# ska-telescope/ska-sdp-screen-fitting

Measured on AMD Instinct MI355X. Metric: screen-slots/sec (ant×time×freq) + FITS-cube wall-clock, KL 256² screen, higher is better.
Workload: dtype f64

## Files before the change

include/screenfit.h:

```cpp
#ifndef SCREENFIT_H
#define SCREENFIT_H

#include <stddef.h>
#include <stdint.h>

#ifdef __cplusplus
extern "C" {
#endif

#define SF_OK 0
#define SF_EINVAL (-22)
#define SF_ENOMEM (-12)
#define SF_EIO (-5)
#define SF_ENODEV (-19)

#define SF_MAX_DIR 60
#define SF_MAX_FIT_DIR 128
#define SF_MAX_EVAL_DIR 128

#define SF_SCREEN_PHASE 0
#define SF_SCREEN_TEC 1
#define SF_SCREEN_AMPLITUDE 2

#define SF_EVAL_NAN_SCRUB 1u
// ... 32 lines not shown
#define SF_OPT_EVAL_XCD_MAP 7
#define SF_OPT_EVAL_GROUPS 8
#define SF_OPT_EVAL_BANDS 9
#define SF_OPT_FIT_LEAN 10
#define SF_OPT_TESS_SLOTS 11
#define SF_OPT_TESS_WAVES 12
#define SF_OPT_TESS_TILE 13
#define SF_OPT_TESS_BOX 14
#define SF_OPT_EVAL_INT 15
#define SF_OPT_EVAL_WG_WAVES 16
#define SF_OPT_FIT_EIG_WAVES 17
#define SF_OPT_FIT_SUBSET_DELETION 18
#define SF_OPT_FIT_WIDE_CACHE 19
#define SF_OPT_FIT_WIDE_POOL_MB 20
#define SF_OPT_FIT_WIDE_POOL_MAX 21
#define SF_EVAL_KERNEL_AUTO 0
#define SF_EVAL_KERNEL_TILE 1
#define SF_EVAL_KERNEL_LDS4 2
#define SF_EVAL_KERNEL_LDS8 3
#define SF_EVAL_KERNEL_LDS16 4
#define SF_EVAL_KERNEL_LDS8H 5
#define SF_EVAL_KERNEL_LDS16H 6
#define SF_EVAL_KERNEL_TILE3 7
#define SF_EVAL_KERNEL_SHB 8
#define SF_EVAL_KERNEL_WIDE 9
int sf_get_eval_kernel(sf_ctx* ctx, int gain, unsigned flags, int* kernel);
#define SF_EVAL_CONTRACTION_F64 0
#define SF_EVAL_CONTRACTION_I8_DIGITS 1
int sf_get_eval_contraction(sf_ctx* ctx, int gain, unsigned flags, int* contraction);
int sf_set_option(sf_ctx* ctx, int option, int value);
// ... 6 lines not shown
                 double beta);
int sf_set_basis_wide(sf_ctx* ctx, const double* pp_host, int D, double r0,
                      double beta);
int sf_get_basis(sf_ctx* ctx, double* c_host, double* pinv_c_host,
                 double* u_host, double* eig_host);

int sf_set_piercepoints(sf_ctx* ctx, const double* pp_host, int D, double r0,
                        double beta);

int sf_kl_fit(sf_ctx* ctx, const double* phase, const float* weight, int T,
              int F, int A, const int* station_order_host,
              const sf_fit_params* params, double* coef, double* resid,
              float* w_out, int32_t* order_out);

int sf_get_fit_stats(sf_ctx* ctx, int* n_masks, int* n_general);

int sf_get_fit_pool(sf_ctx* ctx, uint64_t* masks_host, double* entries_host,
                    int max_masks, int* n_masks);
int sf_get_fit_pool_wide(sf_ctx* ctx, uint64_t* masks_host, double* entries_host,
                         int max_masks, int* n_masks);

int sf_set_grid(sf_ctx* ctx, const double* x_host, int nx,
                const double* y_host, int ny);

int sf_kl_eval(sf_ctx* ctx, const double* coef, int64_t S, float* out,
               int64_t ring_slots, unsigned flags);

int sf_kl_eval_gain(sf_ctx* ctx, const double* coef_phase,
                    const double* coef_xx, const double* coef_yy, int64_t S,
                    float* out, int64_t ring_slots, unsigned flags);
// ... 42 lines not shown
```

ska-sdp-screen-fitting_amd/csrc/capi.hip:

```cpp
#include <hip/hip_runtime.h>

#include <algorithm>
#include <cmath>
#include <cstring>
#include <string>
#include <vector>

#include "sf_internal.h"

namespace sf {
static thread_local std::string g_last_error;
void set_error(const std::string& msg) { g_last_error = msg; }
}

using sf::set_error;

namespace {

int check_device(int device) {
  int n = 0;
  hipError_t e = hipGetDeviceCount(&n);
  if (e != hipSuccess || n == 0) {
    set_error("no HIP device available");
    return SF_ENODEV;
// ... 105 lines not shown
  hipFree(ctx->d_pfrag);
  hipFree(ctx->d_cdig);
  hipFree(ctx->d_kdig);
  hipFree(ctx->d_kflag);
  if (ctx->kdig_read) (void)hipEventDestroy(ctx->kdig_read);
  hipFree(ctx->d_skip);
  hipFree(ctx->d_st_order);
  hipFree(ctx->d_keys);
  hipFree(ctx->d_ids);
  hipFree(ctx->d_pool_mask);
  hipFree(ctx->d_pool);
  hipFree(ctx->d_pool_status);
  hipFree(ctx->d_pos);
  hipFree(ctx->d_sigma);
  hipFree(ctx->d_class);
  hipFree(ctx->d_counters);
  hipFree(ctx->d_scratch);
  hipFree(ctx->d_wscratch);
  hipFree(ctx->d_oscratch);
  hipFree(ctx->d_gw);
  hipFree(ctx->d_smooth);
  hipFree(ctx->d_tess_tab);
  hipFree(ctx->d_tec_ch);
  hipFree(ctx->d_trash);
  delete ctx;
  return SF_OK;
}

int sf_set_stream(sf_ctx* ctx, void* stream) {
  SF_REQUIRE(ctx, SF_EINVAL, "sf_set_stream: NULL context");
// ... 44 lines not shown
  SF_REQUIRE(ctx, SF_EINVAL, "sf_set_option: NULL context");
  switch (option) {
    case SF_OPT_FIT_GENERAL:
      ctx->force_general = value != 0;
      return SF_OK;
    case SF_OPT_EVAL_KERNEL:
      SF_REQUIRE(value >= SF_EVAL_KERNEL_AUTO && value <= SF_EVAL_KERNEL_WIDE,
                 SF_EINVAL, "sf_set_option: unknown evaluation kernel");
      ctx->eval_kernel = value;
      return SF_OK;
    case SF_OPT_FIT_PACK:
      ctx->fit_pack = value != 0;
      return SF_OK;
    case SF_OPT_FIT_LEAN:
      ctx->fit_lean = value != 0;
      return SF_OK;
    case SF_OPT_EVAL_KS_PAD:
      SF_REQUIRE(value >= 0 && value <= 3, SF_EINVAL,
                 "sf_set_option: k-step padding must be 0..3");
      ctx->eval_ks_pad = value;
      return SF_OK;
    case SF_OPT_EVAL_SLEEP:
      SF_REQUIRE(value >= 0 && value <= 1000, SF_EINVAL,
                 "sf_set_option: eval sleep must be 0..1000");
      ctx->eval_sleep = value;
      return SF_OK;
    case SF_OPT_EVAL_XCD_MAP:
      SF_REQUIRE(value >= -1 && value <= 1, SF_EINVAL,
                 "sf_set_option: XCD map must be -1, 0 or 1");
      ctx->eval_xcd_map = value;
// ... 273 lines not shown
}

int sf_get_fit_stats(sf_ctx* ctx, int* n_masks, int* n_general) {
  SF_REQUIRE(ctx, SF_EINVAL, "sf_get_fit_stats: NULL context");
  int c[sf::kFitCounters] = {};
  SF_HIP(hipSetDevice(ctx->device));
  SF_HIP(hipStreamSynchronize(ctx->stream));
  if (ctx->d_counters)
    SF_HIP(hipMemcpy(c, ctx->d_counters, sizeof(c), hipMemcpyDeviceToHost));
  static_assert(sf::kCntIds == sf::kCntWideDecomp, "n_masks reads one slot");
  if (n_masks) *n_masks = c[sf::kCntIds];
  if (n_general) *n_general = c[sf::kCntSlow];
  return SF_OK;
}

int sf_get_fit_pool(sf_ctx* ctx, uint64_t* masks_host, double* entries_host,
                    int max_masks, int* n_masks) {
  SF_REQUIRE(ctx && n_masks && max_masks >= 0, SF_EINVAL, "sf_get_fit_pool: bad argument");
  SF_REQUIRE(max_masks == 0 || (masks_host && entries_host), SF_EINVAL,
             "sf_get_fit_pool: NULL output");
  SF_REQUIRE(!ctx->wide, SF_EINVAL,
             "sf_get_fit_pool: 64-bit mask keys; above SF_MAX_DIR directions "
             "(sf_set_basis_wide) call sf_get_fit_pool_wide");
  SF_HIP(hipSetDevice(ctx->device));
  SF_HIP(hipStreamSynchronize(ctx->stream));
  int c0 = 0;
  if (ctx->d_counters)
    SF_HIP(hipMemcpy(&c0, ctx->d_counters + sf::kCntIds, sizeof(int),
                     hipMemcpyDeviceToHost));
  const int n = ctx->pool_D == ctx->D && (size_t)c0 <= ctx->pool_cap ? c0 : 0;
// ... 424 lines not shown
```

ska-sdp-screen-fitting_amd/csrc/kl_fit_fast.hip:

```cpp
#include <hip/hip_runtime.h>

#include <cmath>
#include <cstdlib>

#include "kl_fit_pool.h"
#include "kl_fit_steps.h"
#include "sf_internal.h"

namespace sf {

constexpr size_t kLdsBytes = 160 * 1024;
constexpr double kTinyW = kPinvAtol * 1.001;

template <int GW>
__global__ __launch_bounds__(256) void kl_classify_kernel(
    const float* __restrict__ weight, int64_t S, int F, int A, int D,
    const int* __restrict__ st_order, const uint8_t* __restrict__ skip,
    int ref_skip, unsigned long long* __restrict__ keys, int cap,
    int* __restrict__ pos, uint8_t* __restrict__ cls,
    int* __restrict__ counters,
    double* __restrict__ coef, double* __restrict__ resid,
    float* __restrict__ w_out, int32_t* __restrict__ order_out) {
  constexpr int kPerWave = 64 / GW;
  const int l = lane();
  const int g = l / GW;
  const int d = l % GW;
  const int64_t s = ((int64_t)blockIdx.x * (blockDim.x / 64) + threadIdx.x / 64) *
                        kPerWave + g;
  const bool live = s < S && d < D;
  float x = 0.0f;
  if (live) {
    x = weight[s * D + d];
    w_out[s * D + d] = x;
  }
  const unsigned long long bm = __ballot(live && x > 0.0f);
  const unsigned long long bt = __ballot(live && x > 0.0f && (double)x <= kTinyW);
  const unsigned long long gmask = (GW == 64) ? ~0ull : ((1ull << GW) - 1ull);
  const unsigned long long mask = (bm >> (g * GW)) & gmask;
  const bool tiny = ((bt >> (g * GW)) & gmask) != 0ull;
  const float w_first = __shfl(x, g * GW + (mask ? __builtin_ctzll(mask) : 0));
  const unsigned long long bn = __ballot(live && x > 0.0f && x != w_first);
  const bool nonuniform = ((bn >> (g * GW)) & gmask) != 0ull;
  if (s >= S) return;
  const SlotGeom sg(s, F, A);
  const bool skipped = sg.skipped(skip, ref_skip);
  if (live && skipped) {
    coef[s * D + d] = 0.0;
    resid[s * D + d] = 0.0;
  }
  if (d != 0) return;
  if (skipped) {
    cls[s] = 1;
    order_out[s] = 0;
    pos[s] = -2;
    return;
  }
  order_out[s] = st_order[sg.a];
  if (tiny) atomicAdd(counters + kCntSlow, 1);
  else if (nonuniform) atomicAdd(counters + kCntNonUniform, 1);
  cls[s] = tiny ? 2 : 0;
  if (mask == full_mask(D)) pos[s] = -1;
  else if (mask == 0ull) pos[s] = -2;
  else pos[s] = table_insert(keys, cap, mask);
}

struct FastLds {
  const double* U;
  const double* C;
  int cld;
  const double* lam;
  double* Vs;
  double* lams;
  double* G;
  double* M;
  double* vec;
// ... 176 lines not shown

#ifndef SF_FIT_MINW
#define SF_FIT_MINW 4
#endif
template <bool SLOW, int SPW, bool LEAN>
__global__ __launch_bounds__(256, SLOW ? 1 : SF_FIT_MINW) void kl_fit_pass_kernel(
    int it, int niter, int64_t S, int F, int A, int D,
    const double* __restrict__ phase, const double* __restrict__ refph,
    int ref_sub, const double* __restrict__ g_u, const double* __restrict__ g_c,
    const double* __restrict__ g_eig, const int* __restrict__ st_order,
    const uint8_t* __restrict__ cls, int* __restrict__ pos,
    const int* __restrict__ ids, unsigned long long* __restrict__ keys, int cap,
    const double* __restrict__ pool, int pool_cap, int* __restrict__ counters,
    int screen_type, double nsigma, int adjust_order, double* __restrict__ coef,
    double* __restrict__ resid, float* __restrict__ w_out,
    int32_t* __restrict__ order_out) {
#pragma clang fp contract(off)
  extern __shared__ double smem[];
  const int ld = odd_ld(D);
  using G = Group<SPW>;
  using M = FitMath<!SLOW>;
  const G tm;
  constexpr bool CG = SPW == 1;
  const int nwaves = blockDim.x / 64;
  const int nslots = nwaves * SPW;
  const int wv = (threadIdx.x / 64) * SPW + G::index();
  const int d = G::lane();
  double* sU = smem;
  double* sC = CG ? nullptr : sU + D * ld;
  double* sl = sU + (CG ? 1 : 2) * D * ld;
  for (int e = threadIdx.x; e < D * D; e += blockDim.x) {
// ... 13 lines not shown
    L.Vs = L.G = L.M = L.lams = nullptr;
    L.vec = wb;
    L.cs = nullptr;
    L.pr = nullptr;
  } else {
    L.Vs = wb;
    L.G = wb + D * ld;
    L.M = L.G + D * ld;
    L.lams = (SLOW ? L.M + D * ld : L.G + D * ld);
    L.vec = L.lams + 64;
    L.cs = reinterpret_cast<double2*>(L.vec + 6 * 64);
    L.pr = reinterpret_cast<int2*>(L.cs + 64);
  }
  const uint8_t want = SLOW ? 2 : 0;

  for (int64_t s = (int64_t)blockIdx.x * nslots + wv; s < S;
       s += (int64_t)gridDim.x * nslots) {
    if (SLOW && cls[s] != want) continue;
    const uint8_t cl = SLOW ? want : cls[s];
    const int a = (int)(s % A);
    const int p0 = pos[s];
    const int64_t base = s * D;
    double phi_d = 0.0, w_d = 0.0, white_d = 0.0, resid_d = 0.0;
    if (d < D) {
      phi_d = phase_ref(phase, refph, ref_sub, s, a, A, D, d);
      w_d = (double)w_out[base + d];
      white_d = it == 0 ? 0.0 : coef[base + d];
      resid_d = it == 0 ? 0.0 : resid[base + d];
    }
    double order = (double)order_out[s];
    const double station_order = (double)st_order[a];
    if (cl != want) continue;
// ... 150 lines not shown
    if (fabs(sd) > nsigma * sig && w != 0.0f) {
      w = 0.0f;
      w_out[s * D + d] = w;
      changed = true;
    }
    if (w > 0.0f) m |= 1ull << d;
  }
  if (changed) {
    pos[s] = (m == 0ull) ? -2 : (m == full_mask(D) ? -1 : table_insert(keys, cap, m));
  }
}

static int launch_pass(sf_ctx* ctx, bool slow, int it, const sf_fit_params* p,
                       const RefSpec& r, int64_t S, int F, int A,
                       const double* phase, double* coef, double* resid,
                       float* w_out, int32_t* order_out, bool lean) {
  const int D = ctx->D;
  const int spw = !slow && D <= 32 && ctx->fit_pack ? 2 : 1;
  lean = !slow && lean && ctx->fit_lean;
  decltype(&kl_fit_pass_kernel<false, 1, false>) const kernels[3][2] = {
      {kl_fit_pass_kernel<false, 1, false>, kl_fit_pass_kernel<false, 2, false>},
      {kl_fit_pass_kernel<false, 1, true>, kl_fit_pass_kernel<false, 2, true>},
      {kl_fit_pass_kernel<true, 1, false>, kl_fit_pass_kernel<true, 2, false>}};
  const auto kernel = kernels[slow ? 2 : lean][spw - 1];
  const size_t shared = fast_shared_bytes(D, spw == 1);
  const size_t slot = fast_wave_bytes(D, slow, lean);
  int nw = 1, best = 0;
  for (int k = 1; k <= 4; ++k) {
    const size_t per_wg = shared + (size_t)k * spw * slot;
    if (per_wg > kLdsBytes) break;
    const int waves = k * (int)(kLdsBytes / per_wg);
    if (waves > best) {
      best = waves;
      nw = k;
    }
  }
  const size_t shm = shared + (size_t)nw * spw * slot;
  SF_TRY_RC(allow_lds(kernel, shm));
  int64_t blocks = (S + nw * spw - 1) / (nw * spw);
  if (blocks > 16384) blocks = 16384;
  hipLaunchKernelGGL(kernel, dim3((unsigned)blocks), dim3(64 * nw), shm,
                     ctx->stream, it, p->niter, S, F, A, D, phase, r.refph, r.sub,
                     ctx->d_u, ctx->d_c, ctx->d_eig, ctx->d_st_order, ctx->d_class,
                     ctx->d_pos, ctx->d_ids, ctx->d_keys, (int)ctx->table_cap,
                     ctx->d_pool, (int)ctx->pool_cap, ctx->d_counters,
                     p->screen_type, p->nsigma, p->adjust_order, coef, resid, w_out,
                     order_out);
  SF_HIP(hipGetLastError());
  return SF_OK;
}

int launch_block_sigma(sf_ctx* ctx, int T, int F, int A, const double* phase,
                       const RefSpec& r, int screen_type, const double* resid,
                       const float* w_out) {
  hipLaunchKernelGGL(kl_block_sigma_kernel, dim3(F * A), dim3(256), 0,
                     ctx->stream, T, F, A, ctx->D, phase, r.refph, r.sub,
                     ctx->d_skip, r.skip, screen_type, resid, w_out,
                     ctx->d_sigma);
  SF_HIP(hipGetLastError());
  return SF_OK;
}

// ... 39 lines not shown
                              w_out, order_out);
  }
  SF_TRY_RC(fit_buffers(ctx, S, F, A, &resid, &w_out, &order_out));
  if (ctx->slot_cap < (size_t)S)
    SF_TRY_RC(replace_pair(ctx->slot_cap, (size_t)S, &ctx->d_pos, (size_t)S,
                           &ctx->d_class, (size_t)S));
  const size_t tcap = next_pow2((size_t)(2 * p->niter + 2) * (size_t)S + 64, 1);
  if (ctx->table_cap < tcap)
    SF_TRY_RC(replace_pair(ctx->table_cap, tcap, &ctx->d_keys, tcap, &ctx->d_ids, tcap));
  SF_TRY_RC(ensure_pool(ctx, 1024));
  const int cap = (int)ctx->table_cap;
  SF_HIP(hipMemsetAsync(ctx->d_keys, 0, ctx->table_cap * sizeof(unsigned long long),
                        ctx->stream));
  SF_HIP(hipMemsetAsync(ctx->d_ids, 0xff, ctx->table_cap * sizeof(int), ctx->stream));
  SF_HIP(hipMemsetAsync(ctx->d_counters, 0, kFitCounters * sizeof(int), ctx->stream));

  {
    const int gw = D <= 8 ? 8 : D <= 16 ? 16 : D <= 32 ? 32 : 64;
    const int64_t per_block = 4 * (64 / gw);
    const dim3 grid((unsigned)((S + per_block - 1) / per_block));
    const auto classify = gw == 8    ? kl_classify_kernel<8>
                          : gw == 16 ? kl_classify_kernel<16>
                          : gw == 32 ? kl_classify_kernel<32>
                                     : kl_classify_kernel<64>;
    hipLaunchKernelGGL(classify, grid, dim3(256), 0, ctx->stream, weight, S, F, A, D,
                       ctx->d_st_order, ctx->d_skip, r.skip, ctx->d_keys, cap,
                       ctx->d_pos, ctx->d_class, ctx->d_counters, coef, resid, w_out,
                       order_out);
    SF_HIP(hipGetLastError());
  }

  const bool block_flags = p->screen_type != SF_SCREEN_PHASE;
  for (int it = 0; it < p->niter; ++it) {
    int n_slow = 0, n_nonuniform = 0;
    SF_TRY_RC(number_and_decompose(ctx, &n_slow, &n_nonuniform));
    SF_TRY_RC(launch_pass(ctx, false, it, p, r, S, F, A, phase, coef, resid, w_out,
                          order_out, n_nonuniform == 0));
    if (n_slow > 0)
      SF_TRY_RC(launch_pass(ctx, true, it, p, r, S, F, A, phase, coef, resid, w_out,
                            order_out, false));
    if (block_flags && it + 1 < p->niter) {
      SF_TRY_RC(launch_block_sigma(ctx, T, F, A, phase, r, p->screen_type, resid,
                                 w_out));
      hipLaunchKernelGGL(kl_block_flag_kernel, dim3((unsigned)((S + 255) / 256)),
                         dim3(256), 0, ctx->stream, S, F, A, D, phase, r.refph,
                         r.sub, ctx->d_class, p->screen_type, p->nsigma,
                         ctx->d_sigma, resid, w_out, ctx->d_keys, cap,
                         ctx->d_pos);
      SF_HIP(hipGetLastError());
    }
  }
  int err = 0;
  SF_HIP(hipMemcpyAsync(&err, ctx->d_counters + kCntError, sizeof(int),
                        hipMemcpyDeviceToHost, ctx->stream));
  SF_HIP(hipStreamSynchronize(ctx->stream));
// ... 13 lines not shown
```

ska-sdp-screen-fitting_amd/csrc/kl_fit_masks.h:

```cpp
#pragma once

#include <hip/hip_runtime.h>

#include "sf_wave.h"

namespace sf {

__device__ __forceinline__ unsigned long long mix64(unsigned long long x) {
  x ^= x >> 30;
  x *= 0xbf58476d1ce4e5b9ull;
  x ^= x >> 27;
  x *= 0x94d049bb133111ebull;
  x ^= x >> 31;
  return x;
}

__host__ __device__ inline unsigned long long full_mask(int D) {
  return D == 64 ? ~0ull : (1ull << D) - 1ull;
}

inline size_t next_pow2(size_t x, size_t floor) {
  size_t p = floor;
  while (p < x) p <<= 1;
  return p;
}

__device__ __forceinline__ bool wave_in_table(int i, int cap) {
  return i - lane() < cap;
}

__device__ __forceinline__ int number_fresh(bool fresh, int* counter) {
  const unsigned long long nb = __ballot(fresh);
  if (nb == 0ull) return -1;
  int base = 0;
  if (lane() == 0) base = atomicAdd(counter, __popcll(nb));
  base = __shfl(base, 0);
  return fresh ? base + Group<1>::rank(nb) : -1;
}

}
```

ska-sdp-screen-fitting_amd/csrc/kl_fit_pool.h:

```cpp
#pragma once

#include <hip/hip_runtime.h>

#include <algorithm>

#include "kl_fit_masks.h"
#include "kl_fit_steps.h"
#include "sf_internal.h"

namespace sf {

constexpr unsigned long long kEmptyKey = 0ull;

__device__ int table_insert(unsigned long long* keys, int cap,
                            unsigned long long key) {
  int h = (int)(mix64(key) & (unsigned long long)(cap - 1));
  for (int probe = 0; probe < cap; ++probe) {
    unsigned long long prev = keys[h];
    if (prev == kEmptyKey) prev = atomicCAS(keys + h, kEmptyKey, key);
    if (prev == kEmptyKey || prev == key) return h;
    h = (h + 1) & (cap - 1);
  }
  return -3;
}

__device__ int table_find(const unsigned long long* keys, int cap,
                          unsigned long long key) {
  int h = (int)(mix64(key) & (unsigned long long)(cap - 1));
  for (int probe = 0; probe < cap; ++probe) {
    const unsigned long long k = keys[h];
    if (k == key) return h;
    if (k == kEmptyKey) return -1;
    h = (h + 1) & (cap - 1);
  }
  return -1;
}

__global__ __launch_bounds__(256) void kl_assign_kernel(
    const unsigned long long* __restrict__ keys, int cap, int* __restrict__ ids,
// ... 444 lines not shown
```

ska-sdp-screen-fitting_amd/csrc/sf_internal.h:

```cpp
#pragma once

#include <hip/hip_runtime.h>

#include <cstdint>
#include <string>
#include <vector>

#include "screenfit.h"

namespace sf {

void set_error(const std::string& msg);

#define SF_HIP(call)                                                        \
  do {                                                                      \
    hipError_t e_ = (call);                                                 \
    if (e_ != hipSuccess) {                                                 \
      ::sf::set_error(std::string(#call) + ": " + hipGetErrorString(e_));   \
      return SF_EIO;                                                        \
    }                                                                       \
  } while (0)

#define SF_REQUIRE(cond, code, msg) \
  do {                              \
// ... 48 lines not shown
  if (shm > 64 * 1024)
    SF_HIP(hipFuncSetAttribute(reinterpret_cast<const void*>(kernel),
                               hipFuncAttributeMaxDynamicSharedMemorySize, (int)shm));
  return SF_OK;
}

enum FitCounter {
  kCntIds = 0,
  kCntWideDecomp = 0,
  kCntPassStart = 1,
  kCntSlow = 2,
  kCntError = 3,
  kCntNonUniform = 4,
  kCntMaxLevel = 5,
  kCntWideMasks = 6,
};
constexpr int kFitCounters = 8;
enum FitError {
  kErrLookupMiss = 1,
  kErrTableFull = 2,
  kErrLeanNonUniform = 4,
  kErrFullMaskInPool = 8,
};

constexpr int kTiles = 4;
constexpr int kWavePix = 16 * kTiles;
constexpr int kEvalWaves = 4;
constexpr int kBlockPix = kWavePix * kEvalWaves;

constexpr int kDigits = 6;

}
// ... 58 lines not shown
  int* d_st_order = nullptr;
  size_t st_order_cap = 0;
  unsigned long long* d_keys = nullptr;
  int* d_ids = nullptr;
  size_t table_cap = 0;
  unsigned long long* d_pool_mask = nullptr;
  double* d_pool = nullptr;
  int fit_eig_waves = 0;
  int fit_subset_deletion = 1;
  size_t pool_cap = 0;
  uint8_t* d_pool_status = nullptr;
  size_t pool_status_cap = 0;
  int pool_D = 0;
  int* d_pos = nullptr;
  uint8_t* d_class = nullptr;
  double* d_sigma = nullptr;
  size_t sigma_cap = 0;
  size_t slot_cap = 0;
  int* d_counters = nullptr;
  size_t counters_cap = 0;
  double* d_scratch = nullptr;
  size_t scratch_cap = 0;
  float* d_wscratch = nullptr;
  size_t wscratch_cap = 0;
  int32_t* d_oscratch = nullptr;
  size_t oscratch_cap = 0;
  double* d_gw = nullptr;
  size_t gw_cap = 0;
  double gw_sigma = -1.0;
  float* d_trash = nullptr;
// ... 3 lines not shown
  size_t tess_tab_cap = 0;
  int force_general = 0;
  int eval_kernel = SF_EVAL_KERNEL_AUTO;
  int64_t eval_max_blocks = 0;
  int eval_ks_pad = 0;
  int eval_sleep = 0;
  int eval_xcd_map = -1;
  int eval_groups = 0;
  int eval_bands = 0;
  int tess_slots = 0;
  int tess_waves = 0;
  int tess_tile = 0;
  int tess_box = -1;
  int fit_pack = 1;
  int fit_lean = 1;
};

namespace sf {
constexpr int kEvalMaxKS = 15;
constexpr int kEvalWideMaxKS = SF_MAX_EVAL_DIR / 4;
inline bool eval_int_applies(const sf_ctx* ctx, bool gain, unsigned flags,
                             bool out_aligned16) {
  return !gain && ctx->dig_ok && ctx->d_cdig && ctx->eval_int != 0 &&
         (flags & SF_EVAL_FAST_SINCOS) && ctx->n_pix % 4 == 0 && out_aligned16 &&
         ctx->ksteps >= 12 && ctx->ksteps <= kEvalMaxKS;
}

struct RefSpec {
  int sub = -1;
  const double* refph = nullptr;
// ... 60 lines not shown
```

ska-sdp-screen-fitting_amd/ska_sdp_screen_fitting_amd/_lib.py:

```python

import contextlib
import ctypes
import os
import threading

import numpy as np

_HERE = os.path.dirname(os.path.abspath(__file__))
LIB_PATH = os.environ.get("SCREENFIT_LIB", os.path.join(_HERE, "libscreenfit.so"))

SF_SCREEN_PHASE = 0
SF_SCREEN_TEC = 1
SF_SCREEN_AMPLITUDE = 2
SF_EVAL_NAN_SCRUB = 1
SF_EVAL_FAST_SINCOS = 1 << 8
SF_EVAL_NT_STORES = 1 << 9
SF_EVAL_BIG_ENDIAN = 1 << 10
SF_MAX_DIR = 60
SF_MAX_FIT_DIR = 128
SF_MAX_EVAL_DIR = 128
SF_MAX_POINTS = 4096
SF_MAX_TEC_FREQ = 4096
SF_OPT_FIT_GENERAL = 1
SF_OPT_EVAL_KERNEL = 2
# ... 4 lines not shown
SF_OPT_EVAL_XCD_MAP = 7
SF_OPT_EVAL_GROUPS = 8
SF_OPT_EVAL_BANDS = 9
SF_OPT_FIT_LEAN = 10
SF_OPT_TESS_SLOTS = 11
SF_OPT_TESS_WAVES = 12
SF_OPT_TESS_TILE = 13
SF_OPT_TESS_BOX = 14
SF_OPT_EVAL_INT = 15
SF_OPT_EVAL_WG_WAVES = 16
SF_OPT_FIT_EIG_WAVES = 17
SF_OPT_FIT_SUBSET_DELETION = 18
SF_OPT_FIT_WIDE_CACHE = 19
SF_OPT_FIT_WIDE_POOL_MB = 20
SF_OPT_FIT_WIDE_POOL_MAX = 21
SF_EVAL_KERNEL_AUTO = 0
SF_EVAL_KERNEL_TILE = 1
SF_EVAL_KERNEL_LDS4 = 2
SF_EVAL_KERNEL_LDS8 = 3
SF_EVAL_KERNEL_LDS16 = 4
SF_EVAL_KERNEL_LDS8H = 5
SF_EVAL_KERNEL_LDS16H = 6
SF_EVAL_KERNEL_TILE3 = 7
SF_EVAL_KERNEL_SHB = 8
SF_EVAL_KERNEL_WIDE = 9
EVAL_KERNEL_NAMES = {SF_EVAL_KERNEL_TILE: "kl_eval_kernel",
                     SF_EVAL_KERNEL_LDS4: "kl_eval_lds_kernel<4 waves>",
                     SF_EVAL_KERNEL_LDS8: "kl_eval_lds_kernel<8 waves>",
                     SF_EVAL_KERNEL_LDS16: "kl_eval_lds_kernel<16 waves>",
                     SF_EVAL_KERNEL_LDS8H: "kl_eval_lds_kernel<8 waves, 2 tiles>",
                     SF_EVAL_KERNEL_LDS16H: "kl_eval_lds_kernel<16 waves, 2 tiles>",
                     SF_EVAL_KERNEL_TILE3: "kl_eval_kernel<3 waves/SIMD>",
                     SF_EVAL_KERNEL_SHB: "kl_eval_kernel<Cpix in LDS>",
                     SF_EVAL_KERNEL_WIDE: "kl_eval_wide_kernel"}

EXPORTED = (
    "sf_version", "sf_last_error", "sf_create", "sf_destroy", "sf_set_stream",
    "sf_synchronize", "sf_set_option", "sf_get_eval_kernel", "sf_get_eval_contraction", "sf_alloc", "sf_free", "sf_copy_h2d", "sf_copy_d2h",
    "sf_set_basis", "sf_set_basis_wide", "sf_set_piercepoints", "sf_get_basis", "sf_kl_fit", "sf_get_fit_stats", "sf_get_fit_pool",
    "sf_get_fit_pool_wide",
    "sf_stream_create", "sf_stream_destroy", "sf_device_cus",
    "sf_set_grid", "sf_kl_eval", "sf_kl_eval_gain", "sf_kl_eval_sums",
    "sf_tess_fill", "sf_smooth",
    "sf_set_points", "sf_kl_eval_points", "sf_kl_eval_point_values",
    "sf_kl_eval_values",
    "sf_set_tec_freqs", "sf_kl_eval_tec",
    "sf_kl_eval_pol", "sf_tess_fill_pol",
)


_identity = {}


def library_identity(path=None):
# ... 47 lines not shown
            "sf_synchronize": ([vp], c_int),
            "sf_set_option": ([vp, c_int, c_int], c_int),
            "sf_get_eval_kernel": ([vp, c_int, ctypes.c_uint, ip], c_int),
            "sf_get_eval_contraction": ([vp, c_int, ctypes.c_uint, ip], c_int),
            "sf_alloc": ([vp, ctypes.c_size_t, ctypes.POINTER(vp)], c_int),
            "sf_free": ([vp, vp], c_int),
            "sf_copy_h2d": ([vp, vp, vp, ctypes.c_size_t], c_int),
            "sf_copy_d2h": ([vp, vp, vp, ctypes.c_size_t], c_int),
            "sf_set_basis": ([vp, vp, c_int, c_dbl, c_dbl], c_int),
            "sf_set_basis_wide": ([vp, vp, c_int, c_dbl, c_dbl], c_int),
            "sf_set_piercepoints": ([vp, vp, c_int, c_dbl, c_dbl], c_int),
            "sf_get_basis": ([vp, vp, vp, vp, vp], c_int),
            "sf_kl_fit": ([vp, vp, vp, c_int, c_int, c_int, ip,
                           ctypes.POINTER(FitParams), vp, vp, vp, vp], c_int),
            "sf_get_fit_stats": ([vp, ip, ip], c_int),
            "sf_get_fit_pool": ([vp, vp, vp, c_int, ip], c_int),
            "sf_get_fit_pool_wide": ([vp, vp, vp, c_int, ip], c_int),
            "sf_set_grid": ([vp, vp, c_int, vp, c_int], c_int),
            "sf_kl_eval": ([vp, vp, i64, vp, i64, ctypes.c_uint], c_int),
            "sf_stream_create": ([vp, ctypes.POINTER(c_int), c_int,
                                  ctypes.POINTER(vp)], c_int),
            "sf_stream_destroy": ([vp, vp], c_int),
            "sf_device_cus": ([vp, ctypes.POINTER(c_int)], c_int),
            "sf_kl_eval_gain": ([vp, vp, vp, vp, i64, vp, i64, ctypes.c_uint],
                                c_int),
            "sf_kl_eval_sums": ([vp, vp, vp, vp, i64, vp, i64, ctypes.c_uint, vp],
                                c_int),
            "sf_tess_fill": ([vp, vp, c_int, c_int, vp, vp, vp, c_int, i64, vp,
                              i64, c_dbl, ctypes.c_uint], c_int),
            "sf_smooth": ([vp, vp, c_int, c_int, i64, c_dbl, ctypes.c_uint], c_int),
# ... 158 lines not shown
            self.h, self._dev(phase, np.float64, n, "phase"),
            self._dev(weight, np.float32, n, "weight"), int(T), int(F), int(A),
            so.ctypes.data_as(ctypes.POINTER(ctypes.c_int)),
            ctypes.byref(prm), self._dev(coef, np.float64, n, "coef"),
            self._dev(resid, np.float64, n, "resid"),
            self._dev(w_out, np.float32, n, "w_out"),
            self._dev(order_out, np.int32, n // max(self.D, 1), "order_out")),
            "sf_kl_fit")

    def fit_stats(self):
        nm, ng = ctypes.c_int(), ctypes.c_int()
        _check(self.lib.sf_get_fit_stats(self.h, ctypes.byref(nm), ctypes.byref(ng)),
               "sf_get_fit_stats")
        return {"n_masks": nm.value, "n_general": ng.value}

    def fit_pool(self):
        n = ctypes.c_int(0)
        _check(self.lib.sf_get_fit_pool(self.h, None, None, 0, ctypes.byref(n)),
               "sf_get_fit_pool")
        D = self.D
        masks = np.zeros(n.value, np.uint64)
        ent = np.zeros((n.value, D * D + D))
        if n.value:
            _check(self.lib.sf_get_fit_pool(self.h, masks.ctypes.data, ent.ctypes.data,
                                            n.value, ctypes.byref(n)), "sf_get_fit_pool")
        order = np.argsort(masks, kind="stable")
        masks, ent = masks[order], ent[order]
        for k, m in enumerate(masks):
            n = bin(int(m)).count("1")
            u = ent[k, :D * D].reshape(D, D)
# ... 212 lines not shown
```

Before: 6.313 million.

## Fit full-mask phase slots one-per-lane across all iterations in a dedicated kernel

Result: faster. 6.377 million (median of 6 runs) (+1.0%).

```diff
diff --git a/include/screenfit.h b/include/screenfit.h
--- a/include/screenfit.h
+++ b/include/screenfit.h
@@ -70,6 +70,7 @@
 #define SF_OPT_FIT_WIDE_CACHE 19
 #define SF_OPT_FIT_WIDE_POOL_MB 20
 #define SF_OPT_FIT_WIDE_POOL_MAX 21
+#define SF_OPT_FIT_LANE 22
 #define SF_EVAL_KERNEL_AUTO 0
 #define SF_EVAL_KERNEL_TILE 1
 #define SF_EVAL_KERNEL_LDS4 2
@@ -106,6 +107,8 @@
               float* w_out, int32_t* order_out);
 
 int sf_get_fit_stats(sf_ctx* ctx, int* n_masks, int* n_general);
+
+int sf_get_fit_lane_stats(sf_ctx* ctx, int64_t* n_lane, int64_t* n_deferred);
 
 int sf_get_fit_pool(sf_ctx* ctx, uint64_t* masks_host, double* entries_host,
                     int max_masks, int* n_masks);
diff --git a/ska-sdp-screen-fitting_amd/csrc/capi.hip b/ska-sdp-screen-fitting_amd/csrc/capi.hip
--- a/ska-sdp-screen-fitting_amd/csrc/capi.hip
+++ b/ska-sdp-screen-fitting_amd/csrc/capi.hip
@@ -143,6 +143,7 @@
   hipFree(ctx->d_pos);
   hipFree(ctx->d_sigma);
   hipFree(ctx->d_class);
+  hipFree(ctx->d_list);
   hipFree(ctx->d_counters);
   hipFree(ctx->d_scratch);
   hipFree(ctx->d_wscratch);
@@ -217,6 +218,9 @@
       return SF_OK;
     case SF_OPT_FIT_LEAN:
       ctx->fit_lean = value != 0;
+      return SF_OK;
+    case SF_OPT_FIT_LANE:
+      ctx->fit_lane = value != 0;
       return SF_OK;
     case SF_OPT_EVAL_KS_PAD:
       SF_REQUIRE(value >= 0 && value <= 3, SF_EINVAL,
@@ -520,6 +524,18 @@
   return SF_OK;
 }
 
+int sf_get_fit_lane_stats(sf_ctx* ctx, int64_t* n_lane, int64_t* n_deferred) {
+  SF_REQUIRE(ctx, SF_EINVAL, "sf_get_fit_lane_stats: NULL context");
+  int c[sf::kFitCounters] = {};
+  SF_HIP(hipSetDevice(ctx->device));
+  SF_HIP(hipStreamSynchronize(ctx->stream));
+  if (ctx->d_counters)
+    SF_HIP(hipMemcpy(c, ctx->d_counters, sizeof(c), hipMemcpyDeviceToHost));
+  if (n_lane) *n_lane = c[sf::kCntLane];
+  if (n_deferred) *n_deferred = c[sf::kCntLaneDeferred];
+  return SF_OK;
+}
+
 int sf_get_fit_pool(sf_ctx* ctx, uint64_t* masks_host, double* entries_host,
                     int max_masks, int* n_masks) {
   SF_REQUIRE(ctx && n_masks && max_masks >= 0, SF_EINVAL, "sf_get_fit_pool: bad argument");
diff --git a/ska-sdp-screen-fitting_amd/csrc/kl_fit_fast.hip b/ska-sdp-screen-fitting_amd/csrc/kl_fit_fast.hip
--- a/ska-sdp-screen-fitting_amd/csrc/kl_fit_fast.hip
+++ b/ska-sdp-screen-fitting_amd/csrc/kl_fit_fast.hip
@@ -3,6 +3,7 @@
 #include <cmath>
 #include <cstdlib>
 
+#include "kl_fit_lane.h"
 #include "kl_fit_pool.h"
 #include "kl_fit_steps.h"
 #include "sf_internal.h"
@@ -20,7 +21,7 @@
     int* __restrict__ pos, uint8_t* __restrict__ cls,
     int* __restrict__ counters,
     double* __restrict__ coef, double* __restrict__ resid,
-    float* __restrict__ w_out, int32_t* __restrict__ order_out) {
+    float* __restrict__ w_out, int32_t* __restrict__ order_out, int lane_fit) {
   constexpr int kPerWave = 64 / GW;
   const int l = lane();
   const int g = l / GW;
@@ -50,7 +51,7 @@
   }
   if (d != 0) return;
   if (skipped) {
-    cls[s] = 1;
+    cls[s] = kClassSkipped;
     order_out[s] = 0;
     pos[s] = -2;
     return;
@@ -58,7 +59,8 @@
   order_out[s] = st_order[sg.a];
   if (tiny) atomicAdd(counters + kCntSlow, 1);
   else if (nonuniform) atomicAdd(counters + kCntNonUniform, 1);
-  cls[s] = tiny ? 2 : 0;
+  const bool to_lane = lane_fit && !tiny && !nonuniform && mask == full_mask(D);
+  cls[s] = tiny ? kClassSlow : to_lane ? kClassLane : kClassFast;
   if (mask == full_mask(D)) pos[s] = -1;
   else if (mask == 0ull) pos[s] = -2;
   else pos[s] = table_insert(keys, cap, mask);
@@ -265,7 +267,7 @@
     const double* __restrict__ pool, int pool_cap, int* __restrict__ counters,
     int screen_type, double nsigma, int adjust_order, double* __restrict__ coef,
     double* __restrict__ resid, float* __restrict__ w_out,
-    int32_t* __restrict__ order_out) {
+    int32_t* __restrict__ order_out, const long long* __restrict__ list) {
 #pragma clang fp contract(off)
   extern __shared__ double smem[];
   const int ld = odd_ld(D);
@@ -309,8 +311,15 @@
   }
   const uint8_t want = SLOW ? 2 : 0;
 
-  for (int64_t s = (int64_t)blockIdx.x * nslots + wv; s < S;
-       s += (int64_t)gridDim.x * nslots) {
+  const int64_t n_work = list ? (int64_t)counters[kCntList] : S;
+  for (int64_t i = (int64_t)blockIdx.x * nslots + wv; i < n_work;
+       i += (int64_t)gridDim.x * nslots) {
+    int64_t s = i;
+    if (list) {
+      const long long e = list[i];
+      if (list_first(e) > it) continue;
+      s = list_slot(e);
+    }
     if (SLOW && cls[s] != want) continue;
     const uint8_t cl = SLOW ? want : cls[s];
     const int a = (int)(s % A);
@@ -491,7 +500,8 @@
 static int launch_pass(sf_ctx* ctx, bool slow, int it, const sf_fit_params* p,
                        const RefSpec& r, int64_t S, int F, int A,
                        const double* phase, double* coef, double* resid,
-                       float* w_out, int32_t* order_out, bool lean) {
+                       float* w_out, int32_t* order_out, bool lean,
+                       const long long* list) {
   const int D = ctx->D;
   const int spw = !slow && D <= 32 && ctx->fit_pack ? 2 : 1;
   lean = !slow && lean && ctx->fit_lean;
@@ -522,7 +532,7 @@
                      ctx->d_pos, ctx->d_ids, ctx->d_keys, (int)ctx->table_cap,
                      ctx->d_pool, (int)ctx->pool_cap, ctx->d_counters,
                      p->screen_type, p->nsigma, p->adjust_order, coef, resid, w_out,
-                     order_out);
+                     order_out, list);
   SF_HIP(hipGetLastError());
   return SF_OK;
 }
@@ -592,6 +602,9 @@
                         ctx->stream));
   SF_HIP(hipMemsetAsync(ctx->d_ids, 0xff, ctx->table_cap * sizeof(int), ctx->stream));
   SF_HIP(hipMemsetAsync(ctx->d_counters, 0, kFitCounters * sizeof(int), ctx->stream));
+  const bool lane_fit = fit_lane_applies(ctx, p);
+  if (lane_fit) SF_TRY_RC(grow(&ctx->d_list, ctx->list_cap, (size_t)S));
+  long long* const list = lane_fit ? ctx->d_list : nullptr;
 
   {
     const int gw = D <= 8 ? 8 : D <= 16 ? 16 : D <= 32 ? 32 : 64;
@@ -604,7 +617,7 @@
     hipLaunchKernelGGL(classify, grid, dim3(256), 0, ctx->stream, weight, S, F, A, D,
                        ctx->d_st_order, ctx->d_skip, r.skip, ctx->d_keys, cap,
                        ctx->d_pos, ctx->d_class, ctx->d_counters, coef, resid, w_out,
-                       order_out);
+                       order_out, lane_fit ? 1 : 0);
     SF_HIP(hipGetLastError());
   }
 
@@ -612,11 +625,13 @@
   for (int it = 0; it < p->niter; ++it) {
     int n_slow = 0, n_nonuniform = 0;
     SF_TRY_RC(number_and_decompose(ctx, &n_slow, &n_nonuniform));
+    if (it == 0 && lane_fit)
+      SF_TRY_RC(launch_fit_lane(ctx, p, r, S, A, phase, coef, resid, w_out, order_out));
     SF_TRY_RC(launch_pass(ctx, false, it, p, r, S, F, A, phase, coef, resid, w_out,
-                          order_out, n_nonuniform == 0));
+                          order_out, n_nonuniform == 0, list));
     if (n_slow > 0)
       SF_TRY_RC(launch_pass(ctx, true, it, p, r, S, F, A, phase, coef, resid, w_out,
-                            order_out, false));
+                            order_out, false, nullptr));
     if (block_flags && it + 1 < p->niter) {
       SF_TRY_RC(launch_block_sigma(ctx, T, F, A, phase, r, p->screen_type, resid,
                                  w_out));
diff --git a/ska-sdp-screen-fitting_amd/csrc/kl_fit_lane.h b/ska-sdp-screen-fitting_amd/csrc/kl_fit_lane.h
--- /dev/null
+++ b/ska-sdp-screen-fitting_amd/csrc/kl_fit_lane.h
@@ -0,0 +1,35 @@
+#pragma once
+
+#include <cstdint>
+
+#include "sf_internal.h"
+
+namespace sf {
+
+constexpr uint8_t kClassFast = 0, kClassSkipped = 1, kClassSlow = 2, kClassLane = 3;
+
+constexpr int kLaneMinD = 3;
+constexpr int kLaneMaxD = 23;
+
+constexpr int kListPassShift = 56;
+__host__ __device__ inline long long list_entry(int64_t s, int first) {
+  return (long long)s | ((long long)first << kListPassShift);
+}
+__host__ __device__ inline int64_t list_slot(long long e) {
+  return (int64_t)(e & ((1ll << kListPassShift) - 1));
+}
+__host__ __device__ inline int list_first(long long e) {
+  return (int)(e >> kListPassShift);
+}
+
+inline bool fit_lane_applies(const sf_ctx* ctx, const sf_fit_params* p) {
+  return ctx->fit_lane && ctx->fit_pack && !ctx->wide &&
+         p->screen_type == SF_SCREEN_PHASE && ctx->D >= kLaneMinD &&
+         ctx->D <= kLaneMaxD;
+}
+
+int launch_fit_lane(sf_ctx* ctx, const sf_fit_params* p, const RefSpec& r,
+                    int64_t S, int A, const double* phase, double* coef,
+                    double* resid, float* w_out, int32_t* order_out);
+
+}
diff --git a/ska-sdp-screen-fitting_amd/csrc/kl_fit_lane.hip b/ska-sdp-screen-fitting_amd/csrc/kl_fit_lane.hip
--- /dev/null
+++ b/ska-sdp-screen-fitting_amd/csrc/kl_fit_lane.hip
@@ -0,0 +1,356 @@
+#include <hip/hip_runtime.h>
+
+#include <cmath>
+
+#include "kl_fit_lane.h"
+#include "kl_fit_masks.h"
+#include "kl_fit_steps.h"
+#include "sf_internal.h"
+
+#pragma clang fp contract(off)
+
+namespace sf {
+
+using LaneMath = FitMath<false>;
+
+
+template <int D, class Leaf>
+__device__ __forceinline__ void tree_sum3(double (&out)[3], Leaf leaf) {
+  static_assert(D <= 32, "a half-wave of directions");
+  double t5[3] = {0.0, 0.0, 0.0};
+#pragma unroll 1
+  for (int b0 = 0; b0 < 2; ++b0) {
+    double t4[3] = {0.0, 0.0, 0.0};
+#pragma unroll 1
+    for (int b1 = 0; b1 < 2; ++b1) {
+      double t3[3] = {0.0, 0.0, 0.0};
+#pragma unroll 1
+      for (int b2 = 0; b2 < 2; ++b2) {
+        double t2[3] = {0.0, 0.0, 0.0};
+#pragma unroll 1
+        for (int b3 = 0; b3 < 2; ++b3) {
+          double t1[3] = {0.0, 0.0, 0.0};
+#pragma unroll 1
+          for (int b4 = 0; b4 < 2; ++b4) {
+            const int p = b0 + 2 * b1 + 4 * b2 + 8 * b3 + 16 * b4;
+            double x[3] = {0.0, 0.0, 0.0};
+            if (p < D) leaf(p, x);
+#pragma unroll
+            for (int k = 0; k < 3; ++k) t1[k] = b4 == 0 ? x[k] : t1[k] + x[k];
+          }
+#pragma unroll
+          for (int k = 0; k < 3; ++k) t2[k] = b3 == 0 ? t1[k] : t2[k] + t1[k];
+        }
+#pragma unroll
+        for (int k = 0; k < 3; ++k) t3[k] = b2 == 0 ? t2[k] : t3[k] + t2[k];
+      }
+#pragma unroll
+      for (int k = 0; k < 3; ++k) t4[k] = b1 == 0 ? t3[k] : t4[k] + t3[k];
+    }
+#pragma unroll
+    for (int k = 0; k < 3; ++k) t5[k] = b0 == 0 ? t4[k] : t5[k] + t4[k];
+  }
+#pragma unroll
+  for (int k = 0; k < 3; ++k) out[k] = t5[k];
+}
+
+template <int D, int LDX, class T>
+__device__ __forceinline__ void store_rows(T* dst, const double* X, int n_elem,
+                                           unsigned long long rows) {
+  for (int e = lane(); e < n_elem; e += 64) {
+    const int r = e / D, d = e % D;
+    if ((rows >> r) & 1ull) dst[e] = (T)X[d * LDX + r];
+  }
+}
+
+constexpr int kGroups = 16;
+__global__ __launch_bounds__(256) void kl_lane_list_kernel(
+    const uint8_t* __restrict__ cls, int64_t S, int* __restrict__ counters,
+    long long* __restrict__ list) {
+  const int l = lane();
+  const int64_t sb = ((int64_t)blockIdx.x * (blockDim.x / 64) + threadIdx.x / 64) *
+                     (64 * kGroups);
+  if (sb >= S) return;
+  int my_at[kGroups];
+  int n_fast = 0, n_lane = 0;
+#pragma unroll
+  for (int g = 0; g < kGroups; ++g) {
+    const int64_t sg = sb + g * 64 + l;
+    const uint8_t c = sg < S ? cls[sg] : kClassSkipped;
+    const unsigned long long fast_rows = __ballot(c == kClassFast);
+    my_at[g] = c == kClassFast ? n_fast + Group<1>::rank(fast_rows) : -1;
+    n_fast += __popcll(fast_rows);
+    n_lane += __popcll(__ballot(c == kClassLane));
+  }
+  unsigned long long old = 0ull;
+  if (l == 0 && (n_fast | n_lane) != 0)
+    old = atomicAdd(reinterpret_cast<unsigned long long*>(counters + kCntLane),
+                    (unsigned long long)n_lane | ((unsigned long long)n_fast << 32));
+  const int base = (int)(__shfl(old, 0) >> 32);
+#pragma unroll
+  for (int g = 0; g < kGroups; ++g)
+    if (my_at[g] >= 0) list[base + my_at[g]] = list_entry(sb + g * 64 + l, 0);
+}
+
+template <int D>
+__global__ __launch_bounds__(64, 2) void kl_fit_lane_kernel(
+    int niter, int64_t S, int A, const double* __restrict__ phase,
+    const double* __restrict__ refph, int ref_sub,
+    const double* __restrict__ g_u, const double* __restrict__ g_eig,
+    const int* __restrict__ st_order, uint8_t* __restrict__ cls,
+    int* __restrict__ pos, unsigned long long* __restrict__ keys, int cap,
+    int* __restrict__ counters, long long* __restrict__ list, double nsigma,
+    int adjust_order, double* __restrict__ coef, double* __restrict__ resid,
+    float* __restrict__ w_out, int32_t* __restrict__ order_out) {
+  constexpr int LDX = 65;
+  __shared__ double X[D * LDX];
+  __shared__ double sU[D * D + D];
+  __shared__ long long row_tf[64];
+  __shared__ int row_a[64];
+  const int l = lane();
+  const int64_t s0 = (int64_t)blockIdx.x * 64;
+  const int64_t s = s0 + l;
+  const bool mine = s < S && cls[s] == kClassLane;
+  if (__ballot(mine) == 0ull) return;
+  const int n_elem = (int)(S - s0 < 64 ? S - s0 : 64) * D;
+  const int a = (int)(s % A);
+  const double* sLam = sU + D * D;
+  for (int e = l; e < D * D; e += 64) sU[e] = g_u[e];
+  if (l < D) sU[D * D + l] = g_eig[l];
+  row_a[l] = a;
+  row_tf[l] = (long long)(s / A);
+  lds_sync();
+  for (int e = l; e < n_elem; e += 64) {
+    const int r = e / D, d = e % D;
+    double v = phase[s0 * D + e];
+    if (refph) v -= refph[row_tf[r] * D + d];
+    else if (ref_sub >= 0) v -= phase[(s0 + r + (ref_sub - row_a[r])) * D + d];
+    X[d * LDX + r] = v;
+  }
+  lds_sync();
+  double* x = X + l;
+
+  bool run = mine;
+  int defer = -1;
+  if (run) {
+    bool finite = true;
+#pragma unroll 1
+    for (int p = 0; p < D; ++p) finite = finite && __builtin_isfinite(x[p * LDX]);
+    if (!finite) {
+      defer = 0;
+      run = false;
+    }
+  }
+  const bool fitted = run;
+  const double wu = mine ? (double)w_out[s * D] : 1.0;
+  const double station_order = mine ? (double)st_order[a] : 0.0;
+  double order = station_order;
+
+  if (run) {
+    if (order > D - 1) order = D - 1;
+    const int K = (int)order;
+    double v0[D], v1[D];
+#pragma unroll
+    for (int k = 0; k < D; ++k) v0[k] = v1[k] = 0.0;
+#pragma unroll 1
+    for (int p = 0; p < D; ++p) {
+      double sn, cn;
+      LaneMath::sin_cos(x[p * LDX], &sn, &cn);
+      const double rc = wu * cn;
+      const double rs = wu * sn;
+      const double* ur = sU + p * D;
+#pragma unroll
+      for (int k = 0; k < D - 1; ++k) {
+        const double u = ur[k];
+        v0[k] += u * rc;
+        v1[k] += u * rs;
+      }
+    }
+#pragma unroll
+    for (int k = 0; k < D - 1; ++k) {
+      const bool keep = k < K && fabs(sLam[k]) > kPinvAtol;
+      v0[k] = keep ? v0[k] / wu : 0.0;
+      v1[k] = keep ? v1[k] / wu : 0.0;
+    }
+    double sh[D];
+#pragma unroll
+    for (int k = 0; k < D; ++k) sh[k] = 0.0;
+#pragma unroll 1
+    for (int p = 0; p < D; ++p) {
+      const double* ur = sU + p * D;
+      double re = 0.0, im = 0.0;
+#pragma unroll
+      for (int k = 0; k < D - 1; ++k) {
+        const double u = ur[k];
+        re += u * v0[k];
+        im += u * v1[k];
+      }
+      const double screen = LaneMath::arctan2(im, re);
+#pragma unroll
+      for (int k = 0; k < D; ++k) sh[k] += ur[k] * screen;
+    }
+#pragma unroll
+    for (int k = 0; k < D; ++k) {
+      const double lm = sLam[k];
+      const bool keep = fabs(lm) > kPinvAtol;
+      v0[k] = keep ? sh[k] / lm : 0.0;
+      v1[k] = keep ? sh[k] : 0.0;
+    }
+    double* crow = coef + s * D;
+#pragma unroll 1
+    for (int p = 0; p < D; p += 2) {
+      double wh[2] = {0.0, 0.0}, cw[2] = {0.0, 0.0};
+#pragma unroll
+      for (int q = 0; q < 2; ++q) {
+        if (p + q < D) {
+          const double* ur = sU + (p + q) * D;
+#pragma unroll
+          for (int r = 0; r < D; ++r) {
+            const double u = ur[r];
+            wh[q] += u * v0[r];
+            cw[q] += u * v1[r];
+          }
+          x[(p + q) * LDX] = x[(p + q) * LDX] - cw[q];
+        }
+      }
+      if (p + 1 < D) {
+        __builtin_memcpy(crow + p, wh, 16);
+      } else {
+        crow[p] = wh[0];
+      }
+    }
+  }
+
+  lds_sync();
+  store_rows<D, LDX>(resid + s0 * D, X, n_elem, __ballot(fitted));
+  lds_sync();
+
+  constexpr unsigned kFull = D == 32 ? ~0u : (1u << D) - 1u;
+  unsigned um = kFull;
+  bool alive = run;
+  for (int it = 0; it < niter; ++it) {
+    if (__ballot(alive) == 0ull) break;
+    if (alive && it > 0) {
+      const int n_unfl = __popc(um);
+      double o = order;
+      if (o > n_unfl - 1) o = n_unfl - 1;
+      if (adjust_order) {
+        double r[3];
+        tree_sum3<D>(r, [&](int p, double(&v)[3]) {
+          const bool unfl = (um >> p) & 1u;
+          double sn = 0.0, cn = 0.0;
+          if (unfl) LaneMath::sin_cos(x[p * LDX], &sn, &cn);
+          const double ww = unfl ? wu : 0.0;
+          v[0] = ww;
+          v[1] = sn * sn * ww;
+          v[2] = cn * cn * ww;
+        });
+        const double m1 = r[1] / r[0];
+        const double m2 = r[2] / r[0];
+        const double redchi2 = (1.0 - hypot(m1, m2)) * r[0] / (n_unfl - o);
+        OrderWalk walk;
+        double moved = o;
+        if (!walk.template step<LaneMath>(0, redchi2, n_unfl, station_order, moved)) {
+          defer = it;
+          alive = false;
+        }
+      }
+      if (alive) order = o;
+    }
+    if (alive && it + 1 < niter) {
+      const auto wrapped = [&](int p) {
+        double r = LaneMath::mod(x[p * LDX], 2.0 * M_PI);
+        if (r < -M_PI) r += 2.0 * M_PI;
+        if (r > M_PI) r -= 2.0 * M_PI;
+        return r;
+      };
+      double t[3];
+      tree_sum3<D>(t, [&](int p, double(&v)[3]) {
+        const double r = wrapped(p);
+        const bool inc = ((um >> p) & 1u) && !isnan(r);
+        double sn = 0.0, cn = 0.0;
+        if (inc) LaneMath::sin_cos(r, &sn, &cn);
+        v[0] = inc ? 1.0 : 0.0;
+        v[1] = sn;
+        v[2] = cn;
+      });
+      const double ms = t[1] / t[0];
+      const double mc = t[2] / t[0];
+      const double stdv = sqrt(-2.0 * LaneMath::ln(hypot(ms, mc)));
+      const double thr = nsigma * stdv;
+      unsigned outl = 0u;
+#pragma unroll 1
+      for (int p = 0; p < D; ++p)
+        if (fabs(wrapped(p)) > thr) outl |= 1u << p;
+      if (outl) {
+        um &= ~outl;
+        int np = -2;
+        if (um != 0u) {
+          np = table_insert(keys, cap, (unsigned long long)um);
+          if (np == -3) atomicOr(counters + kCntError, kErrTableFull);
+        }
+        pos[s] = np;
+        if (um == 0u) alive = false;
+      }
+    }
+  }
+
+  lds_sync();
+  const bool lost = fitted && um != kFull;
+  if (lost) {
+#pragma unroll 1
+    for (int p = 0; p < D; ++p) x[p * LDX] = ((um >> p) & 1u) ? wu : 0.0;
+  }
+  lds_sync();
+  store_rows<D, LDX>(w_out + s0 * D, X, n_elem, __ballot(lost));
+  if (fitted) order_out[s] = (int32_t)order;
+  const int dat = number_fresh(defer >= 0, counters + kCntList);
+  if (defer >= 0) {
+    cls[s] = kClassFast;
+    list[dat] = list_entry(s, defer);
+  }
+  const unsigned long long nd = __ballot(defer >= 0);
+  if (l == 0 && nd != 0ull) atomicAdd(counters + kCntLaneDeferred, __popcll(nd));
+}
+
+template <int D>
+static void launch_lane(sf_ctx* ctx, const sf_fit_params* p, const RefSpec& r,
+                        int64_t S, int A, const double* phase, double* coef,
+                        double* resid, float* w_out, int32_t* order_out) {
+  hipLaunchKernelGGL(kl_fit_lane_kernel<D>, dim3((unsigned)((S + 63) / 64)), dim3(64), 0,
+                     ctx->stream, p->niter, S, A, phase, r.refph, r.sub, ctx->d_u,
+                     ctx->d_eig, ctx->d_st_order, ctx->d_class, ctx->d_pos, ctx->d_keys,
+                     (int)ctx->table_cap, ctx->d_counters, ctx->d_list, p->nsigma,
+                     p->adjust_order, coef, resid, w_out, order_out);
+}
+
+int launch_fit_lane(sf_ctx* ctx, const sf_fit_params* p, const RefSpec& r,
+                    int64_t S, int A, const double* phase, double* coef,
+                    double* resid, float* w_out, int32_t* order_out) {
+  const int64_t per_block = 4 * 64 * kGroups;
+  hipLaunchKernelGGL(kl_lane_list_kernel, dim3((unsigned)((S + per_block - 1) / per_block)),
+                     dim3(256), 0, ctx->stream, ctx->d_class, S, ctx->d_counters,
+                     ctx->d_list);
+  SF_HIP(hipGetLastError());
+#define SF_LANE_CASE(d)                                                        \
+  case d:                                                                      \
+    launch_lane<d>(ctx, p, r, S, A, phase, coef, resid, w_out, order_out);     \
+    break;
+  switch (ctx->D) {
+    SF_LANE_CASE(3) SF_LANE_CASE(4) SF_LANE_CASE(5) SF_LANE_CASE(6)
+    SF_LANE_CASE(7) SF_LANE_CASE(8) SF_LANE_CASE(9) SF_LANE_CASE(10)
+    SF_LANE_CASE(11) SF_LANE_CASE(12) SF_LANE_CASE(13) SF_LANE_CASE(14)
+    SF_LANE_CASE(15) SF_LANE_CASE(16) SF_LANE_CASE(17) SF_LANE_CASE(18)
+    SF_LANE_CASE(19) SF_LANE_CASE(20) SF_LANE_CASE(21) SF_LANE_CASE(22)
+    SF_LANE_CASE(23)
+    default:
+      set_error("sf_kl_fit: no lane kernel for this number of directions");
+      return SF_EINVAL;
+  }
+#undef SF_LANE_CASE
+  static_assert(kLaneMinD == 3 && kLaneMaxD == 23, "the cases above");
+  SF_HIP(hipGetLastError());
+  return SF_OK;
+}
+
+}
diff --git a/ska-sdp-screen-fitting_amd/csrc/kl_fit_masks.h b/ska-sdp-screen-fitting_amd/csrc/kl_fit_masks.h
--- a/ska-sdp-screen-fitting_amd/csrc/kl_fit_masks.h
+++ b/ska-sdp-screen-fitting_amd/csrc/kl_fit_masks.h
@@ -25,6 +25,20 @@
   return p;
 }
 
+constexpr unsigned long long kEmptyKey = 0ull;
+
+__device__ inline int table_insert(unsigned long long* keys, int cap,
+                            unsigned long long key) {
+  int h = (int)(mix64(key) & (unsigned long long)(cap - 1));
+  for (int probe = 0; probe < cap; ++probe) {
+    unsigned long long prev = keys[h];
+    if (prev == kEmptyKey) prev = atomicCAS(keys + h, kEmptyKey, key);
+    if (prev == kEmptyKey || prev == key) return h;
+    h = (h + 1) & (cap - 1);
+  }
+  return -3;
+}
+
 __device__ __forceinline__ bool wave_in_table(int i, int cap) {
   return i - lane() < cap;
 }
diff --git a/ska-sdp-screen-fitting_amd/csrc/kl_fit_pool.h b/ska-sdp-screen-fitting_amd/csrc/kl_fit_pool.h
--- a/ska-sdp-screen-fitting_amd/csrc/kl_fit_pool.h
+++ b/ska-sdp-screen-fitting_amd/csrc/kl_fit_pool.h
@@ -9,20 +9,6 @@
 #include "sf_internal.h"
 
 namespace sf {
-
-constexpr unsigned long long kEmptyKey = 0ull;
-
-__device__ int table_insert(unsigned long long* keys, int cap,
-                            unsigned long long key) {
-  int h = (int)(mix64(key) & (unsigned long long)(cap - 1));
-  for (int probe = 0; probe < cap; ++probe) {
-    unsigned long long prev = keys[h];
-    if (prev == kEmptyKey) prev = atomicCAS(keys + h, kEmptyKey, key);
-    if (prev == kEmptyKey || prev == key) return h;
-    h = (h + 1) & (cap - 1);
-  }
-  return -3;
-}
 
 __device__ int table_find(const unsigned long long* keys, int cap,
                           unsigned long long key) {
diff --git a/ska-sdp-screen-fitting_amd/csrc/sf_internal.h b/ska-sdp-screen-fitting_amd/csrc/sf_internal.h
--- a/ska-sdp-screen-fitting_amd/csrc/sf_internal.h
+++ b/ska-sdp-screen-fitting_amd/csrc/sf_internal.h
@@ -86,8 +86,11 @@
   kCntNonUniform = 4,
   kCntMaxLevel = 5,
   kCntWideMasks = 6,
-};
-constexpr int kFitCounters = 8;
+  kCntLaneDeferred = 7,
+  kCntLane = 8,
+  kCntList = 9,
+};
+constexpr int kFitCounters = 12;
 enum FitError {
   kErrLookupMiss = 1,
   kErrTableFull = 2,
@@ -176,6 +179,8 @@
   int pool_D = 0;
   int* d_pos = nullptr;
   uint8_t* d_class = nullptr;
+  long long* d_list = nullptr;
+  size_t list_cap = 0;
   double* d_sigma = nullptr;
   size_t sigma_cap = 0;
   size_t slot_cap = 0;
@@ -209,6 +214,7 @@
   int tess_box = -1;
   int fit_pack = 1;
   int fit_lean = 1;
+  int fit_lane = 1;
 };
 
 namespace sf {
diff --git a/ska-sdp-screen-fitting_amd/ska_sdp_screen_fitting_amd/_lib.py b/ska-sdp-screen-fitting_amd/ska_sdp_screen_fitting_amd/_lib.py
--- a/ska-sdp-screen-fitting_amd/ska_sdp_screen_fitting_amd/_lib.py
+++ b/ska-sdp-screen-fitting_amd/ska_sdp_screen_fitting_amd/_lib.py
@@ -42,6 +42,7 @@
 SF_OPT_FIT_WIDE_CACHE = 19
 SF_OPT_FIT_WIDE_POOL_MB = 20
 SF_OPT_FIT_WIDE_POOL_MAX = 21
+SF_OPT_FIT_LANE = 22
 SF_EVAL_KERNEL_AUTO = 0
 SF_EVAL_KERNEL_TILE = 1
 SF_EVAL_KERNEL_LDS4 = 2
@@ -65,7 +66,7 @@
 EXPORTED = (
     "sf_version", "sf_last_error", "sf_create", "sf_destroy", "sf_set_stream",
     "sf_synchronize", "sf_set_option", "sf_get_eval_kernel", "sf_get_eval_contraction", "sf_alloc", "sf_free", "sf_copy_h2d", "sf_copy_d2h",
-    "sf_set_basis", "sf_set_basis_wide", "sf_set_piercepoints", "sf_get_basis", "sf_kl_fit", "sf_get_fit_stats", "sf_get_fit_pool",
+    "sf_set_basis", "sf_set_basis_wide", "sf_set_piercepoints", "sf_get_basis", "sf_kl_fit", "sf_get_fit_stats", "sf_get_fit_lane_stats", "sf_get_fit_pool",
     "sf_get_fit_pool_wide",
     "sf_stream_create", "sf_stream_destroy", "sf_device_cus",
     "sf_set_grid", "sf_kl_eval", "sf_kl_eval_gain", "sf_kl_eval_sums",
@@ -143,6 +144,7 @@
             "sf_kl_fit": ([vp, vp, vp, c_int, c_int, c_int, ip,
                            ctypes.POINTER(FitParams), vp, vp, vp, vp], c_int),
             "sf_get_fit_stats": ([vp, ip, ip], c_int),
+            "sf_get_fit_lane_stats": ([vp, ctypes.POINTER(i64), ctypes.POINTER(i64)], c_int),
             "sf_get_fit_pool": ([vp, vp, vp, c_int, ip], c_int),
             "sf_get_fit_pool_wide": ([vp, vp, vp, c_int, ip], c_int),
             "sf_set_grid": ([vp, vp, c_int, vp, c_int], c_int),
@@ -331,6 +333,12 @@
                "sf_get_fit_stats")
         return {"n_masks": nm.value, "n_general": ng.value}
 
+    def fit_lane_stats(self):
+        nl, nd = ctypes.c_int64(), ctypes.c_int64()
+        _check(self.lib.sf_get_fit_lane_stats(self.h, ctypes.byref(nl), ctypes.byref(nd)),
+               "sf_get_fit_lane_stats")
+        return {"n_lane": nl.value, "n_deferred": nd.value}
+
     def fit_pool(self):
         n = ctypes.c_int(0)
         _check(self.lib.sf_get_fit_pool(self.h, None, None, 0, ctypes.byref(n)),
```
